# DavidPetrus/ood_object_detection

Hardware: AMD Instinct MI355X
Metric: images/sec, tf_efficientdet_d0 640px bf16 inference + OOD score (DetBenchPredict end-to-end) (higher is better)
Workload: dtype bf16; 1 GPU; tf_efficientdet_d0 640x640 batch=64/GPU C=90, DetBenchPredict: backbone+BiFPN+heads+OOD energy/max-logit+top-k(5000)+decode+hard NMS; global_batch=64, parallelism=image-sharded dp1, no collective, weights=seeded reference init, randomised BN stats, class bias 0, launch=hipgraph, images_in_flight=192

## Files before the change

### ood_object_detection_amd/csrc/mbconv_wide.hip

```cpp
#include "common.h"

namespace {

struct WideArgs {
    const void* X; void* Y; const void* W1;
    const float* s1; const float* t1; const float* taps; const float* s2; const float* t2;
    float* pool_partial;
    int B, H, W, Cin, mid, Ho, Wo, pad_t, pad_l;
    int TWo, nstrips, band_rows, nbands, IWs, nw, ngroups, ring_bytes, per_image;
    int xpitch, xslot_bytes, pieces_row, ppr, x_off, ring_off, lds_bytes;
    FastDiv fd_ppr;
    int* err_word;
};

#ifndef WIDE_SPIN_LIMIT
#define WIDE_SPIN_LIMIT (1 << 22)
#endif
constexpr int WIDE_HDR = 64 + 1024;

template <int KS, int S, int NKC, int MT, int NO, int NPL, typename T>
__global__ __launch_bounds__((IsPair<T>::value ? 512 : 1024), (IsPair<T>::value ? 2 : 4)) void mbconv_wide_kernel(WideArgs p) {
    extern __shared__ __attribute__((aligned(16))) char lds[];
    constexpr bool PAIR = IsPair<T>::value;
    constexpr int PB = OpGeom<T>::PIECE, CHB = OpGeom<T>::CHUNK;
    constexpr int PXB = 16 * (int)sizeof(T);
    constexpr int NSX = 2 * S;
    const int lane = threadIdx.x & 63, wave = __builtin_amdgcn_readfirstlane(threadIdx.x >> 6);
    const int frow = lane & 15, kg = lane >> 4;
    const int xcd = blockIdx.x & 7, rr_ = blockIdx.x >> 3;
    const int b = (rr_ / p.per_image) * 8 + xcd;
    if (b >= p.B) return;
    int q_ = rr_ % p.per_image;
    const int group = q_ % p.ngroups; q_ /= p.ngroups;
    const int strip = q_ % p.nstrips, band = q_ / p.nstrips;
    const int c0 = 16 * (group * p.nw + wave);
    const int cbytes = p.Cin * (int)sizeof(T), mid = p.mid;
    int* const cnt = reinterpret_cast<int*>(lds);
    char* const xring = lds + p.x_off;
    char* const ring = lds + p.ring_off + wave * p.ring_bytes;
    constexpr int rowbytes = MT * 16 * PXB;
    constexpr int NTAP = KS * KS, NPAIR = (NTAP + 1) / 2;

    for (int i = threadIdx.x * 16; i < p.lds_bytes; i += blockDim.x * 16) *reinterpret_cast<u32x4*>(lds + i) = u32x4{0u, 0u, 0u, 0u};

    Frag<T> wf[NKC];
    const float rs1 = p.s1[c0 + frow], rs2 = p.s2[c0 + frow];
#pragma unroll
    for (int kc = 0; kc < NKC; ++kc) {
        const int off = kc * CHB + kg * PB;
        wf[kc] = ld_frag<T>(reinterpret_cast<const char*>(p.W1) + (long long)(c0 + frow) * cbytes + (off < cbytes ? off : 0));
    }
    const int hi = kg >> 1;
    const bool dactive = (kg & 1) == (frow >> 3);
    const int dq = (frow & 7) >> 1;
    float tapv[NPAIR];
#pragma unroll
    for (int pr = 0; pr < NPAIR; ++pr) {
        const int t = 2 * pr + hi;
        tapv[pr] = p.taps[(long long)(t < NTAP ? t : 0) * mid + c0 + frow];
    }
    constexpr float ESC = -1.4426950408889634f, EINV = -0.6931471805599453f;
    const f32x4 sh1 = *reinterpret_cast<const f32x4*>(p.t1 + c0 + 4 * kg) * ESC;
    const f32x4 t2v = *reinterpret_cast<const f32x4*>(p.t2 + c0 + 4 * kg);
    f32x4 wv[PAIR ? NTAP : 1];
    if constexpr (PAIR) {
        const f32x4 s2q = *reinterpret_cast<const f32x4*>(p.s2 + c0 + 4 * kg);
#pragma unroll
        for (int t = 0; t < NTAP; ++t) wv[t] = *reinterpret_cast<const f32x4*>(p.taps + (long long)t * mid + c0 + 4 * kg) * (s2q * EINV);
    }
#pragma unroll
    for (int kc = 0; kc < NKC; ++kc) {
        const bool kv = kc * CHB + kg * PB < cbytes;
#pragma unroll
        for (int e = 0; e < 8; ++e) {
            if constexpr (PAIR) {
                const float w = ((float)wf[kc].h[e] + (float)wf[kc].l[e]) * (rs1 * ESC);
                const bf16_t wh = (bf16_t)w;
                wf[kc].h[e] = kv ? wh : (bf16_t)0.f;
                wf[kc].l[e] = kv ? (bf16_t)(w - (float)wh) : (bf16_t)0.f;
            } else {
                wf[kc].v[e] = kv ? (bf16_t)((float)wf[kc].v[e] * (rs1 * ESC)) : (bf16_t)0.f;
            }
        }
    }
    unsigned abits[NPAIR], abitl[PAIR ? NPAIR : 1];
#pragma unroll
    for (int pr = 0; pr < NPAIR; ++pr) {
        const bool on = dactive && 2 * pr + hi < NTAP;
        const float tw_ = tapv[pr] * (rs2 * EINV);
        const bf16_t th_ = (bf16_t)tw_;
        abits[pr] = on ? (unsigned)__builtin_bit_cast(unsigned short, th_) << (16 * (frow & 1)) : 0u;
        if constexpr (PAIR) abitl[pr] = on ? (unsigned)__builtin_bit_cast(unsigned short, (bf16_t)(tw_ - (float)th_)) << (16 * (frow & 1)) : 0u;
    }
    auto diag = [&](int pr, bool opaque) {
        unsigned bits = abits[pr];
        if (opaque) asm volatile("" : "+v"(bits));
        const u32x4 fr = {dq == 0 ? bits : 0u, dq == 1 ? bits : 0u, dq == 2 ? bits : 0u, dq == 3 ? bits : 0u};
        Frag<T> af;
        if constexpr (PAIR) {
            unsigned bl = abitl[pr];
            if (opaque) asm volatile("" : "+v"(bl));
            const u32x4 fl = {dq == 0 ? bl : 0u, dq == 1 ? bl : 0u, dq == 2 ? bl : 0u, dq == 3 ? bl : 0u};
            af.h = __builtin_bit_cast(bf16x8, fr);
            af.l = __builtin_bit_cast(bf16x8, fl);
        } else {
            af.v = __builtin_bit_cast(bf16x8, fr);
        }
        return af;
    };
    constexpr bool ARES = KS == 3;
    Frag<T> afr[ARES ? NPAIR : 1];
    if constexpr (ARES) {
#pragma unroll
        for (int pr = 0; pr < NPAIR; ++pr) afr[pr] = diag(pr, false);
    }

    const int oy_b = band * p.band_rows, oy_e = min(p.Ho, oy_b + p.band_rows);
    const int ox0 = strip * p.TWo, tw = min(p.TWo, p.Wo - ox0);
    const int ix0 = ox0 * S - p.pad_l, iy_top = oy_b * S - p.pad_t;
    constexpr int OOB = 0x7FFFFFF0;
    unsigned cmask[MT];
    float caddc[MT];
#pragma unroll
    for (int t = 0; t < MT; ++t) {
        const int c = 16 * t + frow, ix = ix0 + c;
        const bool inside = c < p.IWs && ix >= 0 && ix < p.W;
        cmask[t] = inside ? 0xFFFFFFFFu : 0u;
        caddc[t] = inside ? 1.f : __builtin_inff();
    }
    const int xlane = frow * p.xpitch + kg * PB;
    const int xtile = 16 * p.xpitch;
    const int xlast = ((NKC - 1) * CHB + kg * PB < cbytes) ? (NKC - 1) * CHB : -kg * PB;
    char* const ring_e = ring + frow * PXB;
    const char* const dl = ring + frow * S * PXB + (PAIR ? kg * 16 : (kg & 1) * (PXB / 2));
    const char* const dlh = dl + hi * PXB;
    const int yoff0 = PAIR ? (ox0 + frow) * mid * 4 + ((c0 + 4 * kg) >> 3) * 32 + ((c0 + 4 * kg) & 7) * 2 : ((ox0 + frow) * mid + c0 + 4 * kg) * 2;
    const bool ylast_ok = 16 * (NO - 1) + frow < tw;
    const float vlast = ylast_ok ? 1.f : 0.f;
    const int yoff_last = ylast_ok ? yoff0 : OOB;
    const __amdgpu_buffer_rsrc_t xrs = __builtin_amdgcn_make_buffer_rsrc(
        const_cast<char*>(reinterpret_cast<const char*>(p.X)) + (long long)b * p.H * p.W * cbytes, 0, p.H * p.W * cbytes, 0x00020000);
    const __amdgpu_buffer_rsrc_t yrs = __builtin_amdgcn_make_buffer_rsrc(
        reinterpret_cast<char*>(p.Y) + (long long)b * p.Ho * p.Wo * mid * (int)sizeof(T), 0, p.Ho * p.Wo * mid * (int)sizeof(T), 0x00020000);

    int sgoff[NPL], sloff[NPL];
    bool smine[NPL];
#pragma unroll
    for (int j = 0; j < NPL; ++j) {
        const int i = (int)threadIdx.x + j * (int)blockDim.x;
        const int px = fdiv(i, p.fd_ppr), piece = i - px * p.ppr;
        const int ix = ix0 + px;
        smine[j] = i < p.pieces_row;
        sgoff[j] = (smine[j] && ix >= 0 && ix < p.W) ? ix * cbytes + piece * 16 : OOB;
        sloff[j] = smine[j] ? p.x_off + px * p.xpitch + piece * 16 : 64 + lane * 16;
    }
    u32x4 xs[S][NPL];
    auto issue = [&](int rel, u32x4 (&dst)[NPL]) {
        int iy = iy_top + rel;
        iy = iy < 0 ? 0 : (iy >= p.H ? p.H - 1 : iy);
        const int rowoff = iy * p.W * cbytes;
#pragma unroll
        for (int j = 0; j < NPL; ++j) dst[j] = __builtin_amdgcn_raw_buffer_load_b128(xrs, sgoff[j], rowoff, 0);
    };
    auto commit = [&](int rel, const u32x4 (&src)[NPL]) {
        const int so = (rel & (NSX - 1)) * p.xslot_bytes;
#pragma unroll
        for (int j = 0; j < NPL; ++j) *reinterpret_cast<u32x4*>(lds + sloff[j] + (smine[j] ? so : 0)) = src[j];
        asm volatile("s_waitcnt lgkmcnt(0)" ::: "memory");
        if (lane == 0) __hip_atomic_fetch_add(cnt + (rel & (NSX - 1)), 1, __ATOMIC_RELAXED, __HIP_MEMORY_SCOPE_WORKGROUP);
    };
    auto poll = [&](int rel) {
        const int target = p.nw * (rel / NSX + 1);
        int* c = cnt + (rel & (NSX - 1));
        bool arrived = false;
#pragma unroll 1
        for (int spin = 0; spin < WIDE_SPIN_LIMIT; ++spin) {
            const int v = __builtin_amdgcn_readfirstlane(__hip_atomic_load(c, __ATOMIC_RELAXED, __HIP_MEMORY_SCOPE_WORKGROUP));
            if (v >= target) { arrived = true; break; }
            __builtin_amdgcn_s_sleep(1);
        }
        if (!arrived && lane == 0 && p.err_word != nullptr)
            __hip_atomic_fetch_or(p.err_word, 1, __ATOMIC_RELAXED, __HIP_MEMORY_SCOPE_SYSTEM);
        asm volatile("" ::: "memory");
    };
    auto expand_row = [&](int rel, int slot_bytes) {
        const int iy = iy_top + rel;
        if (iy < 0 || iy >= p.H) {
#pragma unroll
            for (int t = 0; t < MT; ++t) {
                if constexpr (PAIR) *reinterpret_cast<f32x4*>(ring_e + slot_bytes + 16 * PXB * t + kg * 16) = f32x4{0.f, 0.f, 0.f, 0.f};
                else row_store4<T>(ring_e + slot_bytes + 16 * PXB * t, 4 * kg, f32x4{0.f, 0.f, 0.f, 0.f});
            }
            return;
        }
        const char* xb = xring + (rel & (NSX - 1)) * p.xslot_bytes + xlane;
        Frag<T> xf[NKC];
#pragma unroll
        for (int kc = 0; kc < NKC; ++kc) xf[kc] = ld_frag<T>(xb + (kc + 1 < NKC ? kc * CHB : xlast));
#pragma unroll
        for (int t = 0; t < MT; ++t) {
            f32x4 acc = sh1;
#pragma unroll
            for (int kc = 0; kc < NKC; ++kc) mma_chunk(wf[kc], xf[kc], acc);
            if (t + 1 < MT) {
                xb += xtile;
#pragma unroll
                for (int kc = 0; kc < NKC; ++kc) xf[kc] = ld_frag<T>(xb + (kc + 1 < NKC ? kc * CHB : xlast));
            }
            __builtin_amdgcn_sched_barrier(0);
            if constexpr (PAIR) {
                const f32x4 a_ = silu4_scaled(acc, 1.f);
                const unsigned cm = cmask[t];
                const float e0 = a_[0], e1 = a_[1], e2 = a_[2], e3 = a_[3];
                const f32x4 ev = {__builtin_bit_cast(float, __builtin_bit_cast(unsigned, e0) & cm), __builtin_bit_cast(float, __builtin_bit_cast(unsigned, e1) & cm),
                                  __builtin_bit_cast(float, __builtin_bit_cast(unsigned, e2) & cm), __builtin_bit_cast(float, __builtin_bit_cast(unsigned, e3) & cm)};
                *reinterpret_cast<f32x4*>(ring_e + slot_bytes + 16 * PXB * t + kg * 16) = ev;
            } else {
                row_store4<T>(ring_e + slot_bytes + 16 * PXB * t, 4 * kg, silu4_scaled(acc, caddc[t]));
            }
            __builtin_amdgcn_sched_barrier(0);
        }
    };
    auto event = [&](int rel, int slot_bytes, u32x4 (&regs)[NPL]) {
        poll(rel);
        expand_row(rel, slot_bytes);
        commit(rel + S, regs);
        issue(rel + 2 * S, regs);
    };

    __syncthreads();
#pragma unroll
    for (int r = 0; r < S; ++r) { issue(r, xs[r]); commit(r, xs[r]); }
#pragma unroll
    for (int r = 0; r < S; ++r) issue(S + r, xs[r]);
    int next_rel = 0;
#pragma unroll
    for (int r = 0; r < KS - S; ++r) { event(r, r * rowbytes, xs[r % S]); }
    next_rel = KS - S;

    float pl[4] = {0.f, 0.f, 0.f, 0.f};
    int yrow = oy_b * p.Wo * mid * (int)sizeof(T);
    const int ypitch = p.Wo * mid * (int)sizeof(T);
    const int ytile = 16 * mid * (int)sizeof(T);
    int oy = oy_b;
    auto step = [&](auto PHC) {
        constexpr int PH = decltype(PHC)::value;
#pragma unroll
        for (int r = 0; r < S; ++r) event(next_rel + r, ((PH + KS - S + r) % KS) * rowbytes, xs[(KS - S + r) % S]);
        next_rel += S;
        __builtin_amdgcn_sched_barrier(0);
        int hsel = hi;
        asm volatile("" : "+v"(hsel));
        f32x4 acc[NO];
#pragma unroll
        for (int u = 0; u < NO; ++u) acc[u] = t2v;
        if constexpr (PAIR) {
#pragma unroll
            for (int dy = 0; dy < KS; ++dy) {
                f32x4 e[KS][NO];
#pragma unroll
                for (int dx = 0; dx < KS; ++dx)
#pragma unroll
                    for (int u = 0; u < NO; ++u)
                        e[dx][u] = *reinterpret_cast<const f32x4*>(dl + ((PH + dy) % KS) * rowbytes + dx * PXB + u * (16 * S * PXB));
#pragma unroll
                for (int dx = 0; dx < KS; ++dx)
#pragma unroll
                    for (int u = 0; u < NO; ++u) acc[u] = e[dx][u] * wv[dy * KS + dx] + acc[u];
                __builtin_amdgcn_sched_barrier(0);
            }
        }
        constexpr int G = 12 / NO < NPAIR ? 12 / NO : NPAIR;
#pragma unroll
        for (int p0 = 0; p0 < (PAIR ? 0 : NPAIR); p0 += G) {
            Frag<T> bq[G][NO];
#pragma unroll
            for (int g = 0; g < G; ++g) {
                const int pr = p0 + g;
                if (pr < NPAIR) {
                    const int ta = 2 * pr, tb = 2 * pr + 1 < NTAP ? 2 * pr + 1 : 2 * pr;
                    const int offa = ((PH + ta / KS) % KS) * rowbytes + (ta % KS) * PXB;
                    const int offb = ((PH + tb / KS) % KS) * rowbytes + (tb % KS) * PXB;
                    const bool same_row = ta / KS == tb / KS;
                    const char* src = same_row ? dlh + offa : dl + offa + hsel * (offb - offa);
#pragma unroll
                    for (int u = 0; u < NO; ++u) bq[g][u] = ld_frag<T>(src + u * (16 * S * PXB));
                }
            }
#pragma unroll
            for (int g = 0; g < G; ++g) {
                const int pr = p0 + g;
                if (pr < NPAIR) {
                    Frag<T> af;
                    if constexpr (ARES) af = afr[pr]; else af = diag(pr, true);
#pragma unroll
                    for (int u = 0; u < NO; ++u) mma_chunk(af, bq[g][u], acc[u]);
                }
            }
            __builtin_amdgcn_sched_barrier(0);
        }
#pragma unroll
        for (int u = 0; u < NO; ++u) {
            const f32x4 ov = silu4_fast(acc[u]);
            const bool last = u == NO - 1;
            if (last) {
#pragma unroll
                for (int r = 0; r < 4; ++r) pl[r] += ov[r] * vlast;
            } else {
#pragma unroll
                for (int r = 0; r < 4; ++r) pl[r] += ov[r];
            }
            const int yo = last ? yoff_last : yoff0;
            if constexpr (PAIR) {
                u32x2 oh, ol;
                pair_split4(ov, oh, ol);
                __builtin_amdgcn_raw_buffer_store_b64(oh, yrs, yo, yrow + u * ytile, 0);
                __builtin_amdgcn_raw_buffer_store_b64(ol, yrs, yo + 16, yrow + u * ytile, 0);
            } else {
                const bf16x4 ob = {(bf16_t)ov[0], (bf16_t)ov[1], (bf16_t)ov[2], (bf16_t)ov[3]};
                __builtin_amdgcn_raw_buffer_store_b64(__builtin_bit_cast(u32x2, ob), yrs, yo, yrow + u * ytile, 0);
            }
        }
        yrow += ypitch;
        ++oy;
    };
#pragma unroll 1
    while (oy < oy_e) {
        if constexpr (KS == 3) {
            step(IntC<0>{});
            if (oy < oy_e) step(IntC<(S) % 3>{});
            if (oy < oy_e) step(IntC<(2 * S) % 3>{});
        } else {
            step(IntC<0>{});
            if (oy < oy_e) step(IntC<(S) % 5>{});
            if (oy < oy_e) step(IntC<(2 * S) % 5>{});
            if (oy < oy_e) step(IntC<(3 * S) % 5>{});
            if (oy < oy_e) step(IntC<(4 * S) % 5>{});
        }
    }
    if (p.pool_partial != nullptr) {
#pragma unroll
        for (int r = 0; r < 4; ++r) {
            float v = pl[r];
            v += __shfl_xor(v, 1, 64); v += __shfl_xor(v, 2, 64); v += __shfl_xor(v, 4, 64); v += __shfl_xor(v, 8, 64);
            pl[r] = v;
        }
        if (frow == 0) {
            float* dst = p.pool_partial + ((long long)b * (p.nstrips * p.nbands) + band * p.nstrips + strip) * mid + c0 + 4 * kg;
            *reinterpret_cast<f32x4*>(dst) = f32x4{pl[0], pl[1], pl[2], pl[3]};
        }
    }
}

typedef void (*WideKernel)(WideArgs);
struct WideGeometry {
    WideKernel kern; int TWo, nstrips, IWs, IWa, band_rows, nbands, nw, ngroups, ring_bytes, nkc, xpitch, xslot_bytes, npl, wg_per_cu; size_t lds;
};

template <int KS, int S, int NKC, int MT, int NO, typename T>
WideKernel wide_kernel_npl(int npl) {
    if constexpr (IsPair<T>::value) {
        switch (npl) {
            case 1: return mbconv_wide_kernel<KS, S, NKC, MT, NO, 1, T>;
            case 2: return mbconv_wide_kernel<KS, S, NKC, MT, NO, 2, T>;
            case 3: return mbconv_wide_kernel<KS, S, NKC, MT, NO, 3, T>;
            case 4: return mbconv_wide_kernel<KS, S, NKC, MT, NO, 4, T>;
            default: return nullptr;
        }
    } else {
        return npl == 1 ? mbconv_wide_kernel<KS, S, NKC, MT, NO, 1, T> : nullptr;
    }
}

template <int KS, int S, int NKC, typename T>
WideKernel wide_kernel_for(int mt, int no, int npl) {
    if constexpr (S == 1) {
        if (mt == 2) return no == 1 ? wide_kernel_npl<KS, S, NKC, 2, 1, T>(npl) : no == 2 ? wide_kernel_npl<KS, S, NKC, 2, 2, T>(npl) : nullptr;
        if (mt == 3) return no == 2 ? wide_kernel_npl<KS, S, NKC, 3, 2, T>(npl) : no == 3 ? wide_kernel_npl<KS, S, NKC, 3, 3, T>(npl) : nullptr;
        if (mt == 4) return no == 3 ? wide_kernel_npl<KS, S, NKC, 4, 3, T>(npl) : no == 4 ? wide_kernel_npl<KS, S, NKC, 4, 4, T>(npl) : nullptr;
    } else {
        if (mt == 2) return no == 1 ? wide_kernel_npl<KS, S, NKC, 2, 1, T>(npl) : nullptr;
        if (mt == 3) return no == 1 ? wide_kernel_npl<KS, S, NKC, 3, 1, T>(npl) : no == 2 ? wide_kernel_npl<KS, S, NKC, 3, 2, T>(npl) : nullptr;
        if (mt == 4) return no == 2 ? wide_kernel_npl<KS, S, NKC, 4, 2, T>(npl) : nullptr;
    }
    return nullptr;
}

template <int KS, int S, typename T>
WideKernel wide_kernel_ks(const WideGeometry& g) {
    WideKernel kern = nullptr;
    const int mt = g.IWa / 16, no = (g.TWo + 15) / 16;
    if constexpr (IsPair<T>::value) {
        if (mt != 2) return nullptr;
        switch (g.nkc) {
            case 3: kern = no == 1 ? wide_kernel_npl<KS, S, 3, 2, 1, T>(g.npl) : (no == 2 && S == 1) ? wide_kernel_npl<KS, S, 3, 2, 2, T>(g.npl) : nullptr; break;
            case 4: kern = no == 1 ? wide_kernel_npl<KS, S, 4, 2, 1, T>(g.npl) : (no == 2 && S == 1) ? wide_kernel_npl<KS, S, 4, 2, 2, T>(g.npl) : nullptr; break;
            case 5: kern = no == 1 ? wide_kernel_npl<KS, S, 5, 2, 1, T>(g.npl) : (no == 2 && S == 1) ? wide_kernel_npl<KS, S, 5, 2, 2, T>(g.npl) : nullptr; break;
            case 6: kern = no == 1 ? wide_kernel_npl<KS, S, 6, 2, 1, T>(g.npl) : (no == 2 && S == 1) ? wide_kernel_npl<KS, S, 6, 2, 2, T>(g.npl) : nullptr; break;
            default: break;
        }
    } else
    switch (g.nkc) {
        case 3: kern = wide_kernel_for<KS, S, 3, T>(mt, no, g.npl); break;
        case 4: kern = wide_kernel_for<KS, S, 4, T>(mt, no, g.npl); break;
        case 5: kern = wide_kernel_for<KS, S, 5, T>(mt, no, g.npl); break;
        case 6: kern = wide_kernel_for<KS, S, 6, T>(mt, no, g.npl); break;
        default: break;
    }
    return kern;
}

WideKernel wide_kernel(const WideGeometry& g, int k, int stride, bool pair) {
    if (pair) {
        if (k == 3) return stride == 1 ? wide_kernel_ks<3, 1, bf16p_t>(g) : wide_kernel_ks<3, 2, bf16p_t>(g);
        return stride == 1 ? wide_kernel_ks<5, 1, bf16p_t>(g) : wide_kernel_ks<5, 2, bf16p_t>(g);
    }
    if (k == 3) return stride == 1 ? wide_kernel_ks<3, 1, bf16_t>(g) : wide_kernel_ks<3, 2, bf16_t>(g);
    return stride == 1 ? wide_kernel_ks<5, 1, bf16_t>(g) : wide_kernel_ks<5, 2, bf16_t>(g);
}

WideGeometry pick_wide(int H, int W, int Cin, int mid, int k, int stride, bool pair = false) {
    WideGeometry g{};
    const int esz = pair ? 4 : 2, pxb = 16 * esz;
    const int cbytes = Cin * esz;
    g.nkc = (Cin + 31) / 32;
    if ((g.nkc < 3 || g.nkc > 6) || mid % 16 || Cin % 8) return g;
    const int Ho = same_out(H, stride), Wo = same_out(W, stride);
    int best_ns = 0;
    for (int ns = 1; ns <= (Wo + 7) / 8; ++ns) {
        const int two = (Wo + ns - 1) / ns;
        if ((ns - 1) * two >= Wo) continue;
        const int iws = (two - 1) * stride + k;
        if (iws > (pair ? 32 : (k == 5 ? 48 : 64))) continue;
        best_ns = ns; g.TWo = two; g.IWs = iws; g.IWa = (iws + 15) / 16 * 16;
        break;
    }
    if (!best_ns) return g;
    g.nstrips = best_ns;
    const int mt = g.IWa / 16, no = (g.TWo + 15) / 16;
    if (mt > 4 || no > 4) return g;
    {
        const double we = stride * mt * (1.0 + 0.06 * g.nkc), wd = no * (1.2 + 0.05 * ((k * k + 1) / 2));
        const double use = (we * g.IWs / (16.0 * mt) + wd * g.TWo / (16.0 * no)) / (we + wd);
        if (use < 0.75 && !pair) return g;
    }
    g.ring_bytes = k * g.IWa * pxb;
    int P = cbytes / 16;
    while (P % 4 != 2) ++P;
    g.xpitch = P * 16;
    g.xslot_bytes = (g.IWs * g.xpitch + 15) / 16 * 16;
    const int nsx = 2 * stride;
    const size_t xbytes = (size_t)nsx * g.xslot_bytes;
    const int tiles = mid / 16;
    const size_t budget = 160 * 1024;
    const int over = ((16 * no - 1) * stride + k) * pxb - g.IWa * pxb;
    const size_t tail_pad = (size_t)((over > 0 ? over : 0) + 64 + 15) / 16 * 16;
    const int npair = (k * k + 1) / 2;
    const double ce = mt * (1.0 + 0.06 * g.nkc), cd = no * (1.2 + 0.05 * npair);
    double best = -1.0;
    for (int d = 2; d <= 16; ++d) {
        if (tiles % d) continue;
        const size_t l = WIDE_HDR + xbytes + (size_t)d * g.ring_bytes + tail_pad;
        if (l > budget) continue;
        const int npl = (g.IWs * (cbytes / 16) + d * 64 - 1) / (d * 64);
        if (npl > (pair ? 4 : 1)) continue;
        int cap = (int)(budget / l);
        const int rcap = (pair ? 8 : 16) / d;
        if (rcap < 1) continue;
        if (cap > rcap) cap = rcap;
        for (int per_cu = 1; per_cu <= cap; ++per_cu) {
            for (int nb = 1; nb <= 4; ++nb) {
                const int rows = (Ho + nb - 1) / nb;
                if (nb > 1 && rows * stride < k) break;
                const int nbe = (Ho + rows - 1) / rows;
                const long long wgs = 64LL * (tiles / d) * g.nstrips * nbe;
                const int L = (int)((wgs + 255) / 256);
                const int conc = L < per_cu ? L : per_cu;
                const int waves = conc * d;
                const double cost = (double)((L + per_cu - 1) / per_cu) * (rows * (stride * ce + cd) + (k - stride) * ce) * (waves > 8 ? waves : 8);
                if (best < 0 || cost < best * 0.999 || (cost < best * 1.001 && d > g.nw)) {
                    best = cost; g.nw = d; g.wg_per_cu = per_cu; g.lds = l; g.nbands = nbe; g.band_rows = rows; g.npl = npl;
                }
            }
        }
    }
    if (best < 0) return g;
    g.ngroups = tiles / g.nw;
    g.kern = wide_kernel(g, k, stride, pair);
    return g;
}

}

int effdet_mbconv_wide_parts(int H, int W, int Cin, int mid, int k, int stride, int pair) {
    const WideGeometry g = pick_wide(H, W, Cin, mid, k, stride, pair != 0);
    return g.kern ? g.nstrips * g.nbands : 0;
}

int effdet_mbconv_wide_launch(hipStream_t st, const void* X, void* Y, const void* W1, const float* s1, const float* t1,
                              const float* taps, const float* s2, const float* t2, float* pool_partial,
                              int B, int H, int W, int Cin, int mid, int k, int stride, int pair, int sym) {
    const WideGeometry g = pick_wide(H, W, Cin, mid, k, stride, pair != 0);
    if (!g.kern) return EFFDET_EINVAL;
    WideArgs r{};
    r.X = X; r.Y = Y; r.W1 = W1; r.s1 = s1; r.t1 = t1; r.taps = taps; r.s2 = s2; r.t2 = t2; r.pool_partial = pool_partial;
    r.B = B; r.H = H; r.W = W; r.Cin = Cin; r.mid = mid; r.Ho = same_out(H, stride); r.Wo = same_out(W, stride);
    r.pad_t = pad_before(H, k, stride, sym); r.pad_l = pad_before(W, k, stride, sym);
    r.TWo = g.TWo; r.nstrips = g.nstrips; r.band_rows = g.band_rows; r.nbands = g.nbands; r.IWs = g.IWs; r.nw = g.nw; r.ngroups = g.ngroups;
    r.ring_bytes = g.ring_bytes; r.per_image = g.nstrips * g.nbands * g.ngroups;
    r.xpitch = g.xpitch; r.xslot_bytes = g.xslot_bytes; r.ppr = Cin * (pair ? 4 : 2) / 16; r.pieces_row = g.IWs * r.ppr;
    r.x_off = WIDE_HDR; r.ring_off = WIDE_HDR + 2 * stride * g.xslot_bytes; r.lds_bytes = (int)g.lds;
    r.fd_ppr = make_fastdiv(r.ppr);
    r.err_word = effdet_device_error_word();
    if (g.lds > 64 * 1024) {
        if (hipFuncSetAttribute(reinterpret_cast<const void*>(g.kern), hipFuncAttributeMaxDynamicSharedMemorySize, 160 * 1024) != hipSuccess)
            return EFFDET_ELAUNCH;
    }
    hipLaunchKernelGGL(g.kern, dim3(((B + 7) / 8) * r.per_image * 8), dim3(g.nw * 64), g.lds, st, r);
    return effdet_check_launch();
}
```

Baseline: 16730 images/sec.

## Decouple pool-partial granularity from band split in wide MBConv kernel

Separates the squeeze-excite pool partial layout (parts) from the launch band split, so each workgroup may process several parts and flush a partial per part. A second cost-model pass, now including a fixed per-workgroup overhead term, picks fewer, taller bands when that is within a small tolerance of the best cost. Fewer bands means less halo recomputation and fewer workgroup startups. The downstream pool reduction keeps its layout because partials are still written per part. The price is a possible loss of parallelism and a per-row flush check inside the kernel.

```diff
diff --git a/ood_object_detection_amd/csrc/mbconv_wide.hip b/ood_object_detection_amd/csrc/mbconv_wide.hip
--- a/ood_object_detection_amd/csrc/mbconv_wide.hip
+++ b/ood_object_detection_amd/csrc/mbconv_wide.hip
@@ -8,6 +8,7 @@
     float* pool_partial;
     int B, H, W, Cin, mid, Ho, Wo, pad_t, pad_l;
     int TWo, nstrips, band_rows, nbands, IWs, nw, ngroups, ring_bytes, per_image;
+    int part_rows, nparts;
     int xpitch, xslot_bytes, pieces_row, ppr, x_off, ring_off, lds_bytes;
     FastDiv fd_ppr;
     int* err_word;
@@ -243,6 +244,25 @@
     const int ypitch = p.Wo * mid * (int)sizeof(T);
     const int ytile = 16 * mid * (int)sizeof(T);
     int oy = oy_b;
+    int part = oy_b / p.part_rows, oy_flush = min(oy_e, oy_b + p.part_rows);
+    auto flush = [&]() {
+        if (p.pool_partial != nullptr) {
+            float v4[4];
+#pragma unroll
+            for (int r = 0; r < 4; ++r) {
+                float v = pl[r];
+                v += __shfl_xor(v, 1, 64); v += __shfl_xor(v, 2, 64); v += __shfl_xor(v, 4, 64); v += __shfl_xor(v, 8, 64);
+                v4[r] = v;
+                pl[r] = 0.f;
+            }
+            if (frow == 0) {
+                float* dst = p.pool_partial + ((long long)b * (p.nstrips * p.nparts) + part * p.nstrips + strip) * mid + c0 + 4 * kg;
+                *reinterpret_cast<f32x4*>(dst) = f32x4{v4[0], v4[1], v4[2], v4[3]};
+            }
+        }
+        ++part;
+        oy_flush = min(oy_e, oy_flush + p.part_rows);
+    };
     auto step = [&](auto PHC) {
         constexpr int PH = decltype(PHC)::value;
 #pragma unroll
@@ -323,6 +343,7 @@
         }
         yrow += ypitch;
         ++oy;
+        if (oy == oy_flush) flush();
     };
 #pragma unroll 1
     while (oy < oy_e) {
@@ -338,23 +359,11 @@
             if (oy < oy_e) step(IntC<(4 * S) % 5>{});
         }
     }
-    if (p.pool_partial != nullptr) {
-#pragma unroll
-        for (int r = 0; r < 4; ++r) {
-            float v = pl[r];
-            v += __shfl_xor(v, 1, 64); v += __shfl_xor(v, 2, 64); v += __shfl_xor(v, 4, 64); v += __shfl_xor(v, 8, 64);
-            pl[r] = v;
-        }
-        if (frow == 0) {
-            float* dst = p.pool_partial + ((long long)b * (p.nstrips * p.nbands) + band * p.nstrips + strip) * mid + c0 + 4 * kg;
-            *reinterpret_cast<f32x4*>(dst) = f32x4{pl[0], pl[1], pl[2], pl[3]};
-        }
-    }
 }
 
 typedef void (*WideKernel)(WideArgs);
 struct WideGeometry {
-    WideKernel kern; int TWo, nstrips, IWs, IWa, band_rows, nbands, nw, ngroups, ring_bytes, nkc, xpitch, xslot_bytes, npl, wg_per_cu; size_t lds;
+    WideKernel kern; int TWo, nstrips, IWs, IWa, band_rows, nbands, part_rows, nparts, nw, ngroups, ring_bytes, nkc, xpitch, xslot_bytes, npl, wg_per_cu; size_t lds;
 };
 
 template <int KS, int S, int NKC, int MT, int NO, typename T>
@@ -485,6 +494,25 @@
         }
     }
     if (best < 0) return g;
+    g.nparts = g.nbands; g.part_rows = g.band_rows;
+    {
+        const double c0 = 31.0;
+        auto alone = [&](int nbw) {
+            const int rows = g.part_rows * (g.nparts / nbw);
+            const long long wgs = 64LL * (tiles / g.nw) * g.nstrips * nbw;
+            const int L = (int)((wgs + 255) / 256);
+            const int conc = L < g.wg_per_cu ? L : g.wg_per_cu;
+            const int waves = conc * g.nw;
+            return (double)((L + g.wg_per_cu - 1) / g.wg_per_cu) * (c0 + (rows < Ho ? rows : Ho) * (stride * ce + cd) + (k - stride) * ce) * (waves > 8 ? waves : 8);
+        };
+        double low = alone(g.nparts);
+        for (int nbw = 1; nbw < g.nparts; ++nbw)
+            if (g.nparts % nbw == 0 && alone(nbw) < low) low = alone(nbw);
+        int nbw = 1;
+        while (g.nparts % nbw || alone(nbw) > 1.03 * low) ++nbw;
+        g.nbands = nbw;
+        g.band_rows = g.part_rows * (g.nparts / nbw);
+    }
     g.ngroups = tiles / g.nw;
     g.kern = wide_kernel(g, k, stride, pair);
     return g;
@@ -494,7 +522,7 @@
 
 int effdet_mbconv_wide_parts(int H, int W, int Cin, int mid, int k, int stride, int pair) {
     const WideGeometry g = pick_wide(H, W, Cin, mid, k, stride, pair != 0);
-    return g.kern ? g.nstrips * g.nbands : 0;
+    return g.kern ? g.nstrips * g.nparts : 0;
 }
 
 int effdet_mbconv_wide_launch(hipStream_t st, const void* X, void* Y, const void* W1, const float* s1, const float* t1,
@@ -507,6 +535,7 @@
     r.B = B; r.H = H; r.W = W; r.Cin = Cin; r.mid = mid; r.Ho = same_out(H, stride); r.Wo = same_out(W, stride);
     r.pad_t = pad_before(H, k, stride, sym); r.pad_l = pad_before(W, k, stride, sym);
     r.TWo = g.TWo; r.nstrips = g.nstrips; r.band_rows = g.band_rows; r.nbands = g.nbands; r.IWs = g.IWs; r.nw = g.nw; r.ngroups = g.ngroups;
+    r.part_rows = g.part_rows; r.nparts = g.nparts;
     r.ring_bytes = g.ring_bytes; r.per_image = g.nstrips * g.nbands * g.ngroups;
     r.xpitch = g.xpitch; r.xslot_bytes = g.xslot_bytes; r.ppr = Cin * (pair ? 4 : 2) / 16; r.pieces_row = g.IWs * r.ppr;
     r.x_off = WIDE_HDR; r.ring_off = WIDE_HDR + 2 * stride * g.xslot_bytes; r.lds_bytes = (int)g.lds;
```

After: 17120 images/sec (median of 6 runs). 1.02x the previous value.
